# DIAGNijmegen/bodyct-dram-emph-subtype

Measured on NVIDIA B200. Metric: CT volumes/sec med3ddram inference, higher is better.
Workload: dtype f16 operands / f32 accumulate

## Files before the change

### bodyct-dram-emph-subtype_b200/csrc/common.h

```cpp
#pragma once
#include <cuda_bf16.h>
#include <cuda_fp16.h>
#include <cuda_runtime.h>
#include <stdarg.h>
#include <stdint.h>
#include <stdio.h>

#include "dram_b200.h"

namespace dram {

void set_error(const char *fmt, ...);

inline int check_cuda(cudaError_t e, const char *what) {
  if (e == cudaSuccess) return DRAM_OK;
  set_error("%s: %s", what, cudaGetErrorString(e));
  return DRAM_E_LAUNCH;
}

#define DRAM_REQUIRE(cond, ...)       \
  do {                                \
    if (!(cond)) {                    \
      ::dram::set_error(__VA_ARGS__); \
      return DRAM_E_ARG;              \
    }                                 \
  } while (0)

#define DRAM_CHECK_LAUNCH(what)                                       \
  do {                                                                \
    int _rc = ::dram::check_cuda(cudaGetLastError(), what);           \
    if (_rc != DRAM_OK) return _rc;                                   \
  } while (0)

inline int ceil_div(int a, int b) { return (a + b - 1) / b; }
inline int64_t ceil_div64(int64_t a, int64_t b) { return (a + b - 1) / b; }

int worklist_build(const uint32_t *bits, int n, int d, int h, int w, int tw, int th, int td, int d_fastest, int radius,
                   uint8_t *flags, int *list, int *count, int total, cudaStream_t st);

int sm_count();
inline int stream_grid(int64_t work_items, int threads, int ctas_per_sm = 8) {
  int64_t want = ceil_div64(work_items, threads);
  int64_t cap = (int64_t)sm_count() * ctas_per_sm;
  if (want < 1) want = 1;
  return (int)(want < cap ? want : cap);
}


#ifdef __CUDACC__
struct LinIdx {
  int i0, i1;
  float w0, w1;
};
__device__ __forceinline__ LinIdx lin_index_ac(int dst, float scale, int in_size) {
  LinIdx r;
  const float real = scale * (float)dst;
  int i0 = (int)real;
  if (i0 > in_size - 1) i0 = in_size - 1;
  r.i0 = i0;
  r.i1 = i0 + ((i0 < in_size - 1) ? 1 : 0);
  float l1 = real - (float)i0;
  l1 = fminf(fmaxf(l1, 0.0f), 1.0f);
  r.w1 = l1;
  r.w0 = 1.0f - l1;
  return r;
}
__device__ __forceinline__ float bilerp_hw(float a, float b, float c, float d, float w0, float w1, float h0, float h1) {
  return __fmaf_rn(h1, __fmaf_rn(w1, d, __fmul_rn(w0, c)), __fmul_rn(h0, __fmaf_rn(w1, b, __fmul_rn(w0, a))));
}
__device__ __forceinline__ float lerp_d(float p0, float p1, float d0, float d1) {
  return __fmaf_rn(d1, p1, __fmul_rn(d0, p0));
}
__host__ __device__ __forceinline__ float ac_scale(int in_size, int out_size) {
  return out_size > 1 ? (float)(in_size - 1) / (float)(out_size - 1) : 0.0f;
}
#endif

}
```

### bodyct-dram-emph-subtype_b200/csrc/conv3d_slab.cu

```cuda
#include <string.h>

#include "conv_plan.h"

namespace dram {

static constexpr int SL_W = 8, SL_H = 16;
__host__ __device__ constexpr int slab_group(int block_n) { return block_n == 128 ? 2 : 4; }
static constexpr int PL_W = SL_W + 2, PL_H = SL_H + 2;
static constexpr int PLANE_BYTES = PL_W * PL_H * 128;
static constexpr int PLANE_PITCH = 23 * 1024;
#ifndef DRAM_SLAB_RING
#define DRAM_SLAB_RING 7
#endif
static constexpr int RING = DRAM_SLAB_RING;
static constexpr int RING_UP = 6;
static constexpr int LP_W = 7, LP_H = 11;
static constexpr int LP_BYTES = LP_W * LP_H * 128;
static constexpr int LP_PITCH = 10 * 1024;
static constexpr int LP_RING = 3;
static constexpr int UP_WARP0 = 7, UP_THREADS = 128;
static constexpr int SL_THREADS = 224;
static constexpr int SL_A_WARP = 4, SL_MMA_WARP = 5, SL_B_WARP = 6;
static constexpr int SL_BLOCK_K = 64;

// ... 84 lines not shown
      mbar_init(plane_empty(s), 1);
    }
    for (int s = 0; s < B_STAGES; ++s) {
      mbar_init(b_full(s), 1);
      mbar_init(b_empty(s), 1);
    }
    for (int a = 0; a < 2; ++a) {
      mbar_init(tmem_full(a), 1);
      mbar_init(tmem_empty(a), 128);
    }
    if (UP)
      for (int s = 0; s < LP_RING; ++s) {
        mbar_init(lp_full(s), 1);
        mbar_init(lp_empty(s), UP_THREADS);
      }
    asm volatile("fence.mbarrier_init.release.cluster;" ::: "memory");
  }
  if (warp == SL_MMA_WARP) tmem_alloc(tmem_slot, Cfg::TMEM_COLS);
  if (warp == SL_A_WARP && lane == 0) {
    prefetch_tensormap(&map_a1);
    prefetch_tensormap(&map_a2);
  }
  if (warp == SL_B_WARP && lane == 0) prefetch_tensormap(&map_w);
  tcgen05_fence_before();
  __syncthreads();
  tcgen05_fence_after();
  uint32_t tmem_base;
  asm volatile("ld.shared.b32 %0, [%1];" : "=r"(tmem_base) : "r"(tmem_slot));
  tmem_base = __shfl_sync(0xffffffffu, tmem_base, 0);

  const int items_total = p.items ? *p.count : p.items_total;
  const int item_begin = (int)(((long long)blockIdx.x * items_total) / gridDim.x);
  const int item_end = (int)(((long long)(blockIdx.x + 1) * items_total) / gridDim.x);
  auto item_at = [&](int i) { return p.items ? __ldg(p.items + i) : i; };
  const bool single_chunk = !UP && p.chunks_total == 1;

  if (warp == SL_A_WARP) {
    if (lane == 0) {
      unsigned seq_end = 0;
      unsigned lseq = 0;
      int prev = -1;
      for (int i = item_begin; i < item_end; ++i) {
        const int item = item_at(i);
        const SlabItem it = decode_item(p, item, Cfg::GROUP);
        const bool reuse = single_chunk && prev == item - 1 && it.g > 0;
        prev = item;
        for (int c = 0; c < p.chunks_total; ++c) {
          const unsigned seq_base = seq_end - (reuse ? 2u : 0u);
          seq_end = seq_base + ITEM_PLANES;
          if (UP && c < p.chunks1) {
            const int zl0 = up_src_lo(it.q0 - 1, p.up_sd, p.Dl);
            const int zl1 = up_src_hi(it.q0 + SL_GROUP, p.D, p.up_sd, p.Dl);
            const int hl0 = up_src_lo(it.h0 - 1, p.up_sh, p.Hl), wl0 = up_src_lo(it.w0 - 1, p.up_sw, p.Wl);
            for (int zl = zl0; zl <= zl1; ++zl, ++lseq) {
              const int ls = lseq % LP_RING;
              mbar_wait(lp_empty(ls), ((lseq / LP_RING) & 1u) ^ 1u);
              mbar_expect_tx(lp_full(ls), LP_BYTES);
              tma_load_5d(lp_addr(ls), &map_a1, lp_full(ls), c * SL_BLOCK_K, wl0, hl0, zl, it.sample);
            }
            for (int j = 0; j < ITEM_PLANES; ++j) {
              const unsigned seq = seq_base + j;
              mbar_wait(plane_empty(seq % RING), ((seq / RING) & 1u) ^ 1u);
            }
            continue;
          }
          for (int j = reuse ? 2 : 0; j < ITEM_PLANES; ++j) {
            const unsigned seq = seq_base + j;
            const int slot = seq % RING;
            mbar_wait(plane_empty(slot), ((seq / RING) & 1u) ^ 1u);
            mbar_expect_tx(plane_full(slot), PLANE_BYTES);
            if (c < p.chunks1)
              tma_load_5d(plane_addr(slot), &map_a1, plane_full(slot), c * SL_BLOCK_K, it.w0 - 1, it.h0 - 1,
                          it.q0 - 1 + j, it.sample);
            else
              tma_load_5d(plane_addr(slot), &map_a2, plane_full(slot), (c - p.chunks1) * SL_BLOCK_K, it.w0 - 1,
                          it.h0 - 1, it.q0 - 1 + j, it.sample);
// ... 9 lines not shown
      for (int i = item_begin; i < item_end; ++i) {
        for (int c = 0; c < p.chunks_total; ++c) {
          for (int hw = 0; hw < 9; ++hw) {
            mbar_wait(b_empty(stage), phase ^ 1u);
            mbar_expect_tx(b_full(stage), Cfg::B_STAGE_BYTES);
#pragma unroll
            for (int blk = 0; blk < 3; ++blk) {
              const int tap = (2 - blk) * 9 + hw;
              tma_load_2d(b_addr(stage) + (uint32_t)(blk * Cfg::B_BLOCK_BYTES), &map_w, b_full(stage),
                          (tap * p.chunks_total + c) * SL_BLOCK_K, 0);
            }
            if (++stage == B_STAGES) {
              stage = 0;
              phase ^= 1u;
            }
          }
        }
      }
    }
    __syncwarp();
  } else if (warp == SL_MMA_WARP) {
    {
      uint32_t idesc[Cfg::MAX_BLK];
#pragma unroll
      for (int nb = 0; nb < Cfg::MAX_BLK; ++nb) idesc[nb] = make_idesc_16bit(128, (nb + 1) * BLOCK_N, p.epi.is_f16);
      const uint64_t desc_a_const = make_sw128_desc_sbo(0u, PL_W * 128, 0);
      const uint64_t desc_b_const = make_sw128_desc(0u);
      int stage = 0;
      uint32_t phase = 0;
      unsigned seq_end = 0;
      int buf = 0;
      uint32_t buf_phase = 0;
      int prev = -1;
      for (int i = item_begin; i < item_end; ++i) {
        const int item = item_at(i);
        const SlabItem it = decode_item(p, item, Cfg::GROUP);
        mbar_wait(tmem_empty(buf), buf_phase ^ 1u);
        tcgen05_fence_after();
        const uint32_t tmem_d0 = tmem_base + (uint32_t)(buf * SL_GROUP * BLOCK_N);
        const bool reuse = single_chunk && prev == item - 1 && it.g > 0;
        const bool next_reuse = single_chunk && i + 1 < item_end && it.g + 1 < p.groups_d && item_at(i + 1) == item + 1;
        prev = item;
        for (int c = 0; c < p.chunks_total; ++c) {
          const unsigned seq_base = seq_end - (reuse ? 2u : 0u);
          seq_end = seq_base + ITEM_PLANES;
          uint64_t da_plane[ITEM_PLANES];
          uint32_t full_bar[ITEM_PLANES], full_par[ITEM_PLANES], empty_bar[ITEM_PLANES];
#pragma unroll
          for (int j = 0; j < ITEM_PLANES; ++j) {
            const unsigned seq = seq_base + j;
            const int slot = seq % RING;
            uint32_t pa = plane_addr(slot);
            if (p.desc_base_offset_mode) pa |= 0u;
            pa = __shfl_sync(0xffffffffu, pa, 0);
            da_plane[j] = desc_a_const | (uint64_t)((pa & 0x3FFFFu) >> 4);
            full_bar[j] = plane_full(slot);
            full_par[j] = (seq / RING) & 1u;
            empty_bar[j] = plane_empty(slot);
          }
          const bool first_chunk = c == 0;
#pragma unroll
          for (int hw = 0; hw < 9; ++hw) {
            constexpr int kRowBytes = 128;
            const int kh = hw / 3, kw = hw - 3 * kh;
            const uint32_t row_off16 = (uint32_t)((kh * PL_W + kw) * kRowBytes) >> 4;
            mbar_wait(b_full(stage), phase);
            tcgen05_fence_after();
            uint32_t bb = b_addr(stage);
            bb = __shfl_sync(0xffffffffu, bb, 0);
            const uint64_t db_stage = desc_b_const | (uint64_t)((bb & 0x3FFFFu) >> 4);
            if (hw == 0) {
#pragma unroll
              for (int j = 0; j < ITEM_PLANES; ++j) {
                mbar_wait(full_bar[j], full_par[j]);
// ... 48 lines not shown
                    const uint64_t db = db_stage + (uint64_t)(((2 - kd_hi) * Cfg::B_BLOCK_BYTES) >> 4);
                    const uint32_t dcol = tmem_d0 + (uint32_t)(t_min * BLOCK_N);
                    umma_bf16(dcol, da + (uint64_t)(2 * k), db + (uint64_t)(2 * k), idesc[nblk - 1], 1u);
                  }
                }
                if (hw == 8) {
#pragma unroll
                  for (int j = 0; j < ITEM_PLANES; ++j)
                    if (j < SL_GROUP || !next_reuse) umma_commit(empty_bar[j]);
                }
                umma_commit(b_empty(stage));
              }
              __syncwarp();
            }
            if (++stage == B_STAGES) {
              stage = 0;
              phase ^= 1u;
            }
          }
        }
        if (elect_one_sync()) umma_commit(tmem_full(buf));
        __syncwarp();
        if (++buf == 2) {
          buf = 0;
          buf_phase ^= 1u;
        }
      }
    }
    __syncwarp();
  } else if (UP && warp >= UP_WARP0) {
    const int tid = threadIdx.x - UP_WARP0 * 32;
    const int is_f16 = p.epi.is_f16;
    unsigned seq_end = 0, lseq_base = 0;
    for (int i = item_begin; i < item_end; ++i) {
      const SlabItem it = decode_item(p, item_at(i), Cfg::GROUP);
      for (int c = 0; c < p.chunks_total; ++c) {
        const unsigned seq_base = seq_end;
        seq_end = seq_base + ITEM_PLANES;
        if (c >= p.chunks1) {
          for (int j = 0; j < ITEM_PLANES; ++j) {
            const unsigned seq = seq_base + j;
            mbar_wait(plane_empty(seq % RING), ((seq / RING) & 1u) ^ 1u);
          }
          continue;
        }
        const int zl0 = up_src_lo(it.q0 - 1, p.up_sd, p.Dl);
        const int zl1 = up_src_hi(it.q0 + SL_GROUP, p.D, p.up_sd, p.Dl);
        const int hl0 = up_src_lo(it.h0 - 1, p.up_sh, p.Hl), wl0 = up_src_lo(it.w0 - 1, p.up_sw, p.Wl);
        int released = zl0;
        for (int j = 0; j < ITEM_PLANES; ++j) {
          const unsigned seq = seq_base + j;
          const int slot = seq % RING;
          const int z = it.q0 - 1 + j;
          const bool zok = z >= 0 && z < p.D;
          mbar_wait(plane_empty(slot), ((seq / RING) & 1u) ^ 1u);
          LinIdx id = {0, 0, 0.0f, 0.0f};
          uint32_t lp0 = 0, lp1 = 0;
          if (zok) {
            id = lin_index_ac(z, p.up_sd, p.Dl);
            for (; released < id.i0; ++released) mbar_arrive(lp_empty((lseq_base + (unsigned)(released - zl0)) % LP_RING));
            const unsigned s0 = lseq_base + (unsigned)(id.i0 - zl0), s1 = lseq_base + (unsigned)(id.i1 - zl0);
            mbar_wait(lp_full(s0 % LP_RING), (s0 / LP_RING) & 1u);
            mbar_wait(lp_full(s1 % LP_RING), (s1 / LP_RING) & 1u);
            lp0 = lp_addr(s0 % LP_RING);
            lp1 = lp_addr(s1 % LP_RING);
          }
          const uint32_t dst0 = plane_addr(slot);
#pragma unroll 1
// ... 17 lines not shown
              lds(lp0 + o00, a0); lds(lp0 + o01, b0); lds(lp0 + o10, c0); lds(lp0 + o11, d0);
              lds(lp1 + o00, a1); lds(lp1 + o01, b1); lds(lp1 + o10, c1); lds(lp1 + o11, d1);
#pragma unroll
              for (int q = 0; q < 4; ++q) {
                const float2 fa0 = unpack2(a0[q], is_f16), fb0 = unpack2(b0[q], is_f16), fc0 = unpack2(c0[q], is_f16),
                             fd0 = unpack2(d0[q], is_f16);
                const float2 fa1 = unpack2(a1[q], is_f16), fb1 = unpack2(b1[q], is_f16), fc1 = unpack2(c1[q], is_f16),
                             fd1 = unpack2(d1[q], is_f16);
                const float x0 = bilerp_hw(fa0.x, fb0.x, fc0.x, fd0.x, iw.w0, iw.w1, ih.w0, ih.w1);
                const float x1 = bilerp_hw(fa1.x, fb1.x, fc1.x, fd1.x, iw.w0, iw.w1, ih.w0, ih.w1);
                const float y0 = bilerp_hw(fa0.y, fb0.y, fc0.y, fd0.y, iw.w0, iw.w1, ih.w0, ih.w1);
                const float y1 = bilerp_hw(fa1.y, fb1.y, fc1.y, fd1.y, iw.w0, iw.w1, ih.w0, ih.w1);
                o[q] = pack2(lerp_d(x0, x1, id.w0, id.w1), lerp_d(y0, y1, id.w0, id.w1), is_f16);
              }
            }
            const uint32_t dst = dst0 + (uint32_t)(r * 128) + (uint32_t)((c16 ^ (r & 7)) << 4);
            asm volatile("st.shared.v4.b32 [%0], {%1, %2, %3, %4};" ::"r"(dst), "r"(o[0]), "r"(o[1]), "r"(o[2]), "r"(o[3])
                         : "memory");
          }
          asm volatile("fence.proxy.async.shared::cta;" ::: "memory");
          asm volatile("bar.sync 1, %0;" ::"n"(UP_THREADS) : "memory");
          if (tid == 0) mbar_arrive(plane_full(slot));
        }
        for (; released <= zl1; ++released) mbar_arrive(lp_empty((lseq_base + (unsigned)(released - zl0)) % LP_RING));
        lseq_base += (unsigned)(zl1 - zl0 + 1);
      }
    }
  } else if (warp < 4) {
    const int row = warp * 32 + lane;
    const int lw = row & (SL_W - 1);
    const int lh = row >> 3;
    int buf = 0;
    uint32_t buf_phase = 0;
    for (int i = item_begin; i < item_end; ++i) {
      const SlabItem it = decode_item(p, item_at(i), Cfg::GROUP);
      const int oh = it.h0 + lh, ow = it.w0 + lw;
      auto res_ptr = [&](int t) {
        const int od = it.q0 + t;
        const bool valid = (od < p.D) && (oh < p.H) && (ow < p.W);
        return residual_row(p.epi, valid, it.sample, od, oh, ow);
      };
      constexpr int GROUPS_PER_PLANE = BLOCK_N / 32;
      ResGroup res = load_residual_group(p.epi, res_ptr(0), 0);
      mbar_wait(tmem_full(buf), buf_phase);
      tcgen05_fence_after();
#pragma unroll 1
      for (int t = 0; t < SL_GROUP; ++t) {
        const int od = it.q0 + t;
        const bool valid = (od < p.D) && (oh < p.H) && (ow < p.W);
        const uint16_t *res_row = res_ptr(t);
        const uint32_t taddr = tmem_base + (uint32_t)((buf * SL_GROUP + t) * BLOCK_N) + ((uint32_t)(warp * 32) << 16);
#pragma unroll 1
        for (int gq = 0; gq < GROUPS_PER_PLANE; ++gq) {
          const int c0 = gq * 32;
          uint32_t v[32];
          tmem_ld_32x32b_x32(taddr + (uint32_t)c0, v);
          ResGroup next;
          if (gq + 1 < GROUPS_PER_PLANE) next = load_residual_group(p.epi, res_row, c0 + 32);
          else next = load_residual_group(p.epi, t + 1 < SL_GROUP ? res_ptr(t + 1) : nullptr, 0);
          tmem_wait_ld();
#ifndef DRAM_SLAB_EXPERIMENT_NO_EPILOGUE
          if (valid) epilogue_group<BLOCK_N == 32>(p.epi, v, c0, it.sample, od, oh, ow, res);
#endif
          res = next;
        }
      }
      tcgen05_fence_before();
      mbar_arrive(tmem_empty(buf));
// ... 385 lines not shown
```

### bodyct-dram-emph-subtype_b200/csrc/decoder_mask.cu

```cuda
#include "common.h"

namespace dram {

__device__ __forceinline__ int first_source(int c, float scale, int out_size, int in_size) {
  if (c <= 0 || scale <= 0.0f) return 0;
  int x = (int)((float)c / scale);
  if (x > out_size - 1) x = out_size - 1;
  while (x > 0 && lin_index_ac(x - 1, scale, in_size).i0 >= c) --x;
  return x;
}

__global__ void __launch_bounds__(256)
support_rows_kernel(const uint8_t *__restrict__ ess, uint32_t *__restrict__ rows, int64_t total, int W, int w,
                    int words, float sw) {
  for (int64_t t = (int64_t)blockIdx.x * blockDim.x + threadIdx.x; t < total; t += (int64_t)gridDim.x * blockDim.x) {
    const int k = (int)(t % words);
    const uint8_t *e = ess + (t / words) * W;
    const int c0 = k * 32;
    uint32_t bits = 0;
    for (int x = first_source(c0 - 1, sw, W, w); x < W; ++x) {
      const LinIdx ix = lin_index_ac(x, sw, w);
      if (ix.i0 > c0 + 31) break;
      if (e[x]) {
        if (ix.i0 >= c0) bits |= 1u << (ix.i0 - c0);
        if (ix.i1 >= c0 && ix.i1 <= c0 + 31) bits |= 1u << (ix.i1 - c0);
      }
    }
    rows[t] = bits;
  }
}

__global__ void __launch_bounds__(256)
support_planes_kernel(const uint32_t *__restrict__ rows, uint32_t *__restrict__ bits, int n, int D, int H, int d,
                      int h, int words, float sd, float sh) {
  const int64_t total = (int64_t)n * d * h * words;
  for (int64_t t = (int64_t)blockIdx.x * blockDim.x + threadIdx.x; t < total; t += (int64_t)gridDim.x * blockDim.x) {
    const int k = (int)(t % words);
    int64_t r = t / words;
    const int y = (int)(r % h);
    r /= h;
    const int z = (int)(r % d);
    const int s = (int)(r / d);
    uint32_t acc = 0;
    for (int Z = first_source(z - 1, sd, D, d); Z < D; ++Z) {
      const LinIdx iz = lin_index_ac(Z, sd, d);
      if (iz.i0 > z) break;
      if (iz.i0 != z && iz.i1 != z) continue;
      for (int Y = first_source(y - 1, sh, H, h); Y < H; ++Y) {
        const LinIdx iy = lin_index_ac(Y, sh, h);
        if (iy.i0 > y) break;
        if (iy.i0 == y || iy.i1 == y) acc |= rows[(((int64_t)s * D + Z) * H + Y) * words + k];
      }
    }
    bits[t] = acc;
  }
}

__global__ void __launch_bounds__(256)
worklist_flags_kernel(const uint32_t *__restrict__ bits, uint8_t *__restrict__ flags, int total, int d, int h, int w,
                      int words, int tw, int th, int td, int d_fastest, int radius) {
  const int tiles_w = (w + tw - 1) / tw, tiles_h = (h + th - 1) / th, tiles_d = (d + td - 1) / td;
  for (int i = blockIdx.x * blockDim.x + threadIdx.x; i < total; i += gridDim.x * blockDim.x) {
    int r = i, iw, ih, id;
    if (d_fastest) {
      id = r % tiles_d; r /= tiles_d;
      iw = r % tiles_w; r /= tiles_w;
      ih = r % tiles_h; r /= tiles_h;
    } else {
      iw = r % tiles_w; r /= tiles_w;
      ih = r % tiles_h; r /= tiles_h;
      id = r % tiles_d; r /= tiles_d;
    }
    const int s = r;
    const int z0 = max(id * td - radius, 0), z1 = min(id * td + td - 1 + radius, d - 1);
    const int y0 = max(ih * th - radius, 0), y1 = min(ih * th + th - 1 + radius, h - 1);
    const int x0 = max(iw * tw - radius, 0), x1 = min(iw * tw + tw - 1 + radius, w - 1);
    const int k0 = x0 >> 5, k1 = x1 >> 5;
    bool on = false;
    for (int z = z0; z <= z1 && !on; ++z)
      for (int y = y0; y <= y1 && !on; ++y) {
        const uint32_t *row = bits + (((int64_t)s * d + z) * h + y) * words;
        for (int k = k0; k <= k1; ++k) {
          uint32_t m = 0xffffffffu;
          if (k == k0) m &= 0xffffffffu << (x0 & 31);
          if (k == k1) m &= 0xffffffffu >> (31 - (x1 & 31));
          if (row[k] & m) {
            on = true;
            break;
          }
        }
      }
    flags[i] = on ? 1 : 0;
  }
}

static constexpr int WL_THREADS = 1024, WL_PER_THREAD = 16;
__global__ void __launch_bounds__(WL_THREADS)
worklist_compact_kernel(const uint8_t *__restrict__ flags, int total, int *__restrict__ list, int *__restrict__ count) {
  __shared__ int warp_sum[WL_THREADS / 32];
  const int lane = threadIdx.x & 31, wid = threadIdx.x >> 5;
  int base = 0;
  for (int start = 0; start < total; start += WL_THREADS * WL_PER_THREAD) {
    const int i0 = start + threadIdx.x * WL_PER_THREAD;
    uint32_t m = 0;
#pragma unroll
    for (int j = 0; j < WL_PER_THREAD; ++j)
      if (i0 + j < total && flags[i0 + j]) m |= 1u << j;
    const int cnt = __popc(m);
    int incl = cnt;
#pragma unroll
    for (int o = 1; o < 32; o <<= 1) {
      const int v = __shfl_up_sync(0xffffffffu, incl, o);
      if (lane >= o) incl += v;
    }
    if (lane == 31) warp_sum[wid] = incl;
    __syncthreads();
    int before = 0, all = 0;
    for (int q = 0; q < WL_THREADS / 32; ++q) {
      const int v = warp_sum[q];
      if (q < wid) before += v;
      all += v;
    }
    int pos = base + before + incl - cnt;
    for (; m; m &= m - 1) list[pos++] = i0 + __ffs(m) - 1;
    base += all;
    __syncthreads();
  }
  if (threadIdx.x == 0) *count = base;
}

int worklist_build(const uint32_t *bits, int n, int d, int h, int w, int tw, int th, int td, int d_fastest, int radius,
                   uint8_t *flags, int *list, int *count, int total, cudaStream_t st) {
  if (!bits || !flags || !list || !count || n <= 0 || d <= 0 || h <= 0 || w <= 0 || total <= 0 || radius < 0) {
    set_error("worklist: null buffer, empty grid or negative radius");
    return DRAM_E_ARG;
  }
  const int words = ceil_div(w, 32);
  worklist_flags_kernel<<<ceil_div(total, 256) < 4096 ? ceil_div(total, 256) : 4096, 256, 0, st>>>(
      bits, flags, total, d, h, w, words, tw, th, td, d_fastest, radius);
  DRAM_CHECK_LAUNCH("worklist_flags_kernel launch");
  worklist_compact_kernel<<<1, WL_THREADS, 0, st>>>(flags, total, list, count);
  DRAM_CHECK_LAUNCH("worklist_compact_kernel launch");
  return DRAM_OK;
}

}

using namespace dram;

extern "C" int dram_decoder_support(const uint8_t *ess, int32_t n, int32_t D, int32_t H, int32_t W, int32_t d,
                                    int32_t h, int32_t w, uint32_t *rows, uint32_t *bits, void *stream) {
  DRAM_REQUIRE(ess && rows && bits, "dram_decoder_support: null pointer");
  DRAM_REQUIRE(n > 0 && D > 0 && H > 0 && W > 0 && d > 0 && h > 0 && w > 0 && d <= D && h <= H && w <= W,
               "dram_decoder_support: bad sizes (%d x %d x %d -> %d x %d x %d)", D, H, W, d, h, w);
  cudaStream_t st = reinterpret_cast<cudaStream_t>(stream);
  const int words = ceil_div(w, 32);
  const int64_t total_rows = (int64_t)n * D * H * words, total_bits = (int64_t)n * d * h * words;
  const int grid_rows = (int)(ceil_div64(total_rows, 256) < 8192 ? ceil_div64(total_rows, 256) : 8192);
  const int grid_bits = (int)(ceil_div64(total_bits, 256) < 8192 ? ceil_div64(total_bits, 256) : 8192);
  support_rows_kernel<<<grid_rows, 256, 0, st>>>(ess, rows, total_rows, W, w, words, ac_scale(w, W));
  DRAM_CHECK_LAUNCH("support_rows_kernel launch");
  support_planes_kernel<<<grid_bits, 256, 0, st>>>(rows, bits, n, D, H, d, h, words, ac_scale(d, D), ac_scale(h, H));
  DRAM_CHECK_LAUNCH("support_planes_kernel launch");
  return DRAM_OK;
}
```

### bodyct-dram-emph-subtype_b200/csrc/upsample_umma.cu

```cuda
#include "umma_common.cuh"

namespace dram {

static constexpr int U_TW = 8, U_TH = 4, U_TD = 4;
static constexpr int U_PW = 6, U_PH = 4, U_PD = 4;
static constexpr int U_K = U_PW * U_PH * U_PD;
static constexpr int U_B_BYTES = U_K * 128;
static constexpr int U_B_STAGES = 6;
static constexpr int U_W_BYTES = 2 * 128 * 128;
static constexpr int U_OUT_BYTES = 128 * 128;
static constexpr int U_ACC = 4;
static constexpr int U_THREADS = 320;
static constexpr int U_PRODUCER_WARP = 4, U_MMA_WARP = 5, U_GEN_WARP0 = 6;
static constexpr int U_SMEM_BYTES = 1024 + U_B_STAGES * U_B_BYTES + 2 * U_W_BYTES + 2 * U_OUT_BYTES + 256;

struct UpParams {
  int n, Dl, Hl, Wl, D, H, W, C;
  int chunks;
  int tiles_w, tiles_h, tiles_d, tiles_per_sample, total_tiles;
  float sd, sh, sw;
  int is_f16;
  const int *items, *count;
};

// ... 38 lines not shown
  auto w_empty = [&](int s) { return bar_base + 8u * (2 * U_B_STAGES + 2 + s); };
  auto t_full = [&](int a) { return bar_base + 8u * (2 * U_B_STAGES + 4 + a); };
  auto t_empty = [&](int a) { return bar_base + 8u * (2 * U_B_STAGES + 4 + U_ACC + a); };
  const uint32_t tmem_slot = bar_base + 8u * (2 * U_B_STAGES + 4 + 2 * U_ACC);

  const int warp = uniform_warp_idx();
  const int lane = threadIdx.x & 31;

  if (threadIdx.x == 0) {
    for (int s = 0; s < U_B_STAGES; ++s) {
      mbar_init(b_full(s), 1);
      mbar_init(b_empty(s), 1);
    }
    for (int s = 0; s < 2; ++s) {
      mbar_init(w_full(s), 128);
      mbar_init(w_empty(s), 1);
    }
    for (int a = 0; a < U_ACC; ++a) {
      mbar_init(t_full(a), 1);
      mbar_init(t_empty(a), 128);
    }
    asm volatile("fence.mbarrier_init.release.cluster;" ::: "memory");
  }
  if (warp == U_MMA_WARP) tmem_alloc(tmem_slot, U_ACC * 64);
  if (warp == U_PRODUCER_WARP && lane == 0) prefetch_tensormap(&map_in);
  if (threadIdx.x == 0) prefetch_tensormap(&map_out);
  tcgen05_fence_before();
  __syncthreads();
  tcgen05_fence_after();
  uint32_t tmem_base;
  asm volatile("ld.shared.b32 %0, [%1];" : "=r"(tmem_base) : "r"(tmem_slot));
  tmem_base = __shfl_sync(0xffffffffu, tmem_base, 0);
  const int total = p.items ? *p.count : p.total_tiles;
  auto tile_at = [&](int i) { return p.items ? __ldg(p.items + i) : i; };

  if (warp == U_PRODUCER_WARP) {
    if (lane == 0) {
      int stage = 0;
      uint32_t phase = 0;
      for (int i = blockIdx.x; i < total; i += gridDim.x) {
        const UpTile t = decode_up_tile(p, tile_at(i));
        for (int c = 0; c < p.chunks; ++c) {
          mbar_wait(b_empty(stage), phase ^ 1u);
          mbar_expect_tx(b_full(stage), U_B_BYTES);
          tma_load_5d(b_addr(stage), &map_in, b_full(stage), c * 64, t.wl0, t.hl0, t.dl0, t.sample);
          if (++stage == U_B_STAGES) {
            stage = 0;
            phase ^= 1u;
          }
        }
      }
    }
    __syncwarp();
  } else if (warp == U_MMA_WARP) {
    const uint32_t idesc = make_idesc_up(64, p.is_f16);
    int stage = 0, acc = 0, wi = 0;
    uint32_t phase = 0, acc_phase = 0, w_phase = 0;
    for (int i = blockIdx.x; i < total; i += gridDim.x) {
      mbar_wait(w_full(wi), w_phase);
      tcgen05_fence_after();
      for (int c = 0; c < p.chunks; ++c) {
        mbar_wait(t_empty(acc), acc_phase ^ 1u);
        mbar_wait(b_full(stage), phase);
        tcgen05_fence_after();
        if (elect_one_sync()) {
#pragma unroll
          for (int j = 0; j < U_K / 16; ++j) {
            const uint64_t da = make_sw128_desc(w_addr(wi) + (uint32_t)((j >> 2) * (128 * 128) + (j & 3) * 32));
            const uint64_t db = make_sw128_desc(b_addr(stage) + (uint32_t)(j * 16 * 128));
            umma_bf16(tmem_base + (uint32_t)(acc * 64), da, db, idesc, j > 0 ? 1u : 0u);
          }
          umma_commit(b_empty(stage));
          umma_commit(t_full(acc));
          if (c == p.chunks - 1) umma_commit(w_empty(wi));
// ... 36 lines not shown
        for (int a = 0; a < 3; ++a)
          if (ix[a].i1 == ix[a].i0) {
            ix[a].w0 += ix[a].w1;
            ix[a].w1 = 0.0f;
          }
#pragma unroll
        for (int cd = 0; cd < 2; ++cd)
#pragma unroll
          for (int chh = 0; chh < 2; ++chh)
#pragma unroll
            for (int cw = 0; cw < 2; ++cw) {
              const float wt = (cd ? ix[0].w1 : ix[0].w0) * ((chh ? ix[1].w1 : ix[1].w0) * (cw ? ix[2].w1 : ix[2].w0));
              if ((cd && ix[0].i1 == ix[0].i0) || (chh && ix[1].i1 == ix[1].i0) || (cw && ix[2].i1 == ix[2].i0)) continue;
              const int zd = (cd ? ix[0].i1 : ix[0].i0) - t.dl0, zh = (chh ? ix[1].i1 : ix[1].i0) - t.hl0;
              const int zw = (cw ? ix[2].i1 : ix[2].i0) - t.wl0;
              const int k = (zd * U_PH + zh) * U_PW + zw;
              const int kk = k & 63;
              const uint32_t addr = base + (uint32_t)((k >> 6) * 128 * 128) + (uint32_t)((((kk >> 3) ^ (r & 7)) << 4) + (kk & 7) * 2);
              unsigned short bits;
              if (p.is_f16) {
                const __half hv = __float2half_rn(wt);
                bits = *reinterpret_cast<const unsigned short *>(&hv);
              } else {
                const __nv_bfloat16 hv = __float2bfloat16_rn(wt);
                bits = *reinterpret_cast<const unsigned short *>(&hv);
              }
              asm volatile("st.shared.u16 [%0], %1;" ::"r"(addr), "h"(bits) : "memory");
              mine[cd * 4 + chh * 2 + cw] = addr;
            }
      }
    };
    int wi = 0;
    uint32_t w_phase = 0;
    for (int i = blockIdx.x; i < total; i += gridDim.x) {
      const UpTile t = decode_up_tile(p, tile_at(i));
      mbar_wait(w_empty(wi), w_phase ^ 1u);
      if (wi == 0) generate(t, w_addr(0), prev0);
      else generate(t, w_addr(1), prev1);
      asm volatile("fence.proxy.async.shared::cta;" ::: "memory");
      mbar_arrive(w_full(wi));
      if (++wi == 2) {
        wi = 0;
        w_phase ^= 1u;
      }
    }
  } else {
    const int row = warp * 32 + lane;
    int acc = 0, gi = 0;
    uint32_t acc_phase = 0;
    for (int i = blockIdx.x; i < total; i += gridDim.x) {
      const UpTile t = decode_up_tile(p, tile_at(i));
      for (int c = 0; c < p.chunks; ++c, ++gi) {
        const int b = gi & 1;
        mbar_wait(t_full(acc), acc_phase);
        tcgen05_fence_after();
        const uint32_t taddr = tmem_base + (uint32_t)(acc * 64) + ((uint32_t)(warp * 32) << 16);
        uint32_t v0[32], v1[32];
        tmem_ld_32x32b_x32(taddr, v0);
        tmem_ld_32x32b_x32(taddr + 32u, v1);
        if (threadIdx.x == 0) tma_store_wait_read<1>();
        asm volatile("bar.sync 1, 128;" ::: "memory");
        tmem_wait_ld();
        tcgen05_fence_before();
        mbar_arrive(t_empty(acc));
        const uint32_t orow = out_addr(b) + (uint32_t)row * 128u;
#pragma unroll
        for (int j = 0; j < 8; ++j) {
          const uint32_t *v = j < 4 ? v0 : v1;
          const int o = (j & 3) * 8;
          const uint32_t chunk = (uint32_t)((j ^ (row & 7)) << 4);
          asm volatile("st.shared.v4.b32 [%0], {%1, %2, %3, %4};" ::"r"(orow + chunk),
                       "r"(pack2(__uint_as_float(v[o + 0]), __uint_as_float(v[o + 1]), p.is_f16)),
                       "r"(pack2(__uint_as_float(v[o + 2]), __uint_as_float(v[o + 3]), p.is_f16)),
                       "r"(pack2(__uint_as_float(v[o + 4]), __uint_as_float(v[o + 5]), p.is_f16)),
                       "r"(pack2(__uint_as_float(v[o + 6]), __uint_as_float(v[o + 7]), p.is_f16))
                       : "memory");
        }
        asm volatile("fence.proxy.async.shared::cta;" ::: "memory");
        asm volatile("bar.sync 1, 128;" ::: "memory");
        if (threadIdx.x == 0) {
          tma_store_5d(&map_out, out_addr(b), c * 64, t.w0, t.h0, t.d0, t.sample);
          tma_store_commit();
        }
        if (++acc == U_ACC) {
// ... 125 lines not shown
```

### bodyct-dram-emph-subtype_b200/engine.py

```python
import os

import torch

from . import ops

LAYER_CFG = ((64, 1, 1), (128, 2, 1), (256, 1, 2), (512, 1, 4))


def _conv_out(n, k, s, d, p):
    return (n + 2 * p - d * (k - 1) - 1) // s + 1


class _Step:

    __slots__ = ("name", "fn", "flops", "executed_flops", "conv_part")

    def __init__(self, name, fn, flops=0, executed_flops=None, conv_part=False):
        self.name, self.fn, self.flops = name, fn, flops
        self.executed_flops = flops if executed_flops is None else executed_flops
        self.conv_part = conv_part or flops > 0


class Med3DEngine:
    def __init__(self, model, batch, dims, device, act_dtype=None):
        if device.type != "cuda":
            raise RuntimeError("Med3DEngine needs a CUDA device: this path has no CPU implementation")
        self.model = model
        self.act_dtype = ops.default_act_dtype() if act_dtype is None else act_dtype
        self.batch, self.dims, self.device = batch, tuple(dims), device
        self.head_kind = model.head_kind
        self._weights = {}
        self._packers = []
        self.steps = []
        self.conv_flops = 0
        self._graph = None
        self._graph_restricted = None
        self._restricted = None
        self._sat_counter = torch.zeros(1, dtype=torch.int32, device=device)
        self._sat_checked_epoch = None
        self.last_saturation_count = None
        self._build()
        self._weights_epoch = model.weights_epoch


    def _register_weight(self, name, pack_fn):
        bufs = tuple(t.to(self.device).contiguous() for t in pack_fn())
        self._weights[name] = bufs

        def refill(bufs=bufs, pack_fn=pack_fn):
            for dst, src in zip(bufs, pack_fn()):
                dst.copy_(src)

        self._packers.append(refill)
# ... 180 lines not shown
        self.us1_g = torch.empty((B, D2, H2, W2, 64), dtype=bf, device=dev)
        self.steps.append(_Step("us1.0.gather_w", lambda: ops.upconv_axis(z, 3, 9, out=self.us1_r), conv_part=True))
        self.steps.append(_Step("us1.0.gather_h", lambda: ops.upconv_axis(self.us1_r, 2, 3, out=self.us1_q), conv_part=True))
        self.steps.append(_Step("us1.0.gather_d", lambda: ops.upconv_axis(self.us1_q, 1, 1, out=self.us1_g), conv_part=True))
        wskip = self._register_weight("us1.0.skip", pack_skip)
        return self._add_conv("us1.0", x1, wskip, residual=self.us1_g).out

    def _launch_steps(self, first=None):
        (first or self.steps[0].fn)()
        self._launch_tail()

    def _launch_tail(self):
        for st in self.steps[1:]:
            st.fn()

    def hu_stem(self, hu, lut, lo=-1150):
        if not hasattr(self, "stem_weights"):
            raise RuntimeError("the int16-HU stem needs the fused stem kernel (DRAM_B200_STEM=unfold is set)")
        if tuple(hu.shape) != (self.batch,) + self.dims:
            raise ValueError(f"hu shape {tuple(hu.shape)} does not match the engine's {(self.batch,) + self.dims}")
        w, b, m = self.stem_weights
        return lambda: ops.stem_conv7_hu(hu, lut, w, b, m, out=self.stem_out, lo=lo)

    def image_stem(self, image):
        if not hasattr(self, "stem_weights"):
            raise RuntimeError("image_stem needs the fused stem kernel (DRAM_B200_STEM=unfold is set)")
        img = image.reshape(self.batch, *self.dims)
        if img.dtype != torch.float32 or not img.is_contiguous():
            raise ValueError("image_stem: expected a contiguous fp32 image")
        w, b, m = self.stem_weights
        return lambda: ops.stem_conv7(img, w, b, m, out=self.stem_out)

    def _restricted_tail(self):
        for fn in self._restricted[2]:
            fn()

    def _support(self, ess):
        if tuple(ess.shape) != (self.batch,) + self.dims or ess.dtype != torch.uint8 or not ess.is_contiguous():
            raise ValueError(f"active_ess: expected contiguous uint8 {(self.batch,) + self.dims}, got "
                             f"{ess.dtype} {tuple(ess.shape)}")
        if self._restricted is None:
            B, (D, H, W), (d, h, w) = self.batch, self.dims, self.half_dims
            words = (w + 31) // 32
            rows = torch.empty((B, D, H, words), dtype=torch.int32, device=self.device)
            support = torch.empty((B, d, h, words), dtype=torch.int32, device=self.device)
            lists, listed = [], {}
            for name, plan, radius, _ in self._decoder:
                size = plan.worklist_size() if plan is not None else 0
                if size == 0:
                    continue
                flags = torch.empty(size, dtype=torch.uint8, device=self.device)
                items = torch.empty(size, dtype=torch.int32, device=self.device)
                count = torch.empty(1, dtype=torch.int32, device=self.device)
                lists.append(lambda plan=plan, r=radius, f=flags, i=items, c=count: plan.build_worklist(support, r, f, i, c))
                listed[name] = lambda plan=plan, i=items, c=count: plan.run_listed(i, c)
            self._restricted = (rows, support, lists + [listed.get(st.name, st.fn) for st in self.steps[1:]])
        rows, support, _ = self._restricted
        ops.decoder_support(ess, self.half_dims, rows=rows, out=support)

    def run_network(self, first=None, active_ess=None):
        if self._weights_epoch != self.model.weights_epoch:
            self.refresh_weights()
        mode = ops.sat_check_mode()
        if self.act_dtype == torch.float16 and (
                mode == "always" or (mode == "first" and self._sat_checked_epoch != self._weights_epoch)):
            lib = ops._capi.load()
            self._sat_counter.zero_()
            ops.check(lib.dram_set_saturation_counter(ops._p(self._sat_counter)), "dram_set_saturation_counter")
            try:
                self._launch_steps(first)
            finally:
                lib.dram_set_saturation_counter(None)
            clamped = int(self._sat_counter.item())
            self.last_saturation_count = clamped
            if clamped:
                raise ops.ActivationOverflow(
                    f"{clamped} 32-channel output groups exceeded the fp16 range (+-65504) and were clamped: this "
                    "checkpoint/input needs bf16 storage (model.act_dtype = torch.bfloat16 or DRAM_B200_DTYPE=bf16)")
            self._sat_checked_epoch = self._weights_epoch
            return self.dense
        tail = self._launch_tail
        if active_ess is not None:
            self._support(active_ess)
            tail = self._restricted_tail
        if not ops.graphs_enabled() or torch.cuda.is_current_stream_capturing():
            (first or self.steps[0].fn)()
            tail()
            return self.dense
        (first or self.steps[0].fn)()
        attr = "_graph" if active_ess is None else "_graph_restricted"
        if getattr(self, attr) is None:
# ... 34 lines not shown
```

Before: 221.6.

## Overlap worklist builds on side stream and parallelise decoder support kernels

The restricted-decoder path now builds its worklists on a side CUDA stream, letting them overlap the encoder steps, and joins the main stream just before the first listed step. The worklist compaction moves from one CTA to a multi-CTA scan. The support-row bitmask kernel now reads the ess mask with vectorised 16-byte loads, skips zero vectors and accumulates bits in shared memory with atomics. Item-list prefetching via a cursor struct and hoisting one loop bound are smaller tweaks. These changes add stream-synchronisation complexity and a dependence on the side stream being captured correctly in graphs.

```diff
diff --git a/bodyct-dram-emph-subtype_b200/csrc/common.h b/bodyct-dram-emph-subtype_b200/csrc/common.h
--- a/bodyct-dram-emph-subtype_b200/csrc/common.h
+++ b/bodyct-dram-emph-subtype_b200/csrc/common.h
@@ -48,6 +48,23 @@
 
 
 #ifdef __CUDACC__
+struct ListCursor {
+  const int *items;
+  int pos, end, stride, cur, nxt;
+  __device__ __forceinline__ int at(int i) const { return i < end ? (items ? __ldg(items + i) : i) : -1; }
+  __device__ __forceinline__ ListCursor(const int *list, int begin, int end_, int stride_ = 1)
+      : items(list), pos(begin), end(end_), stride(stride_) {
+    cur = at(begin);
+    nxt = at(begin + stride_);
+  }
+  __device__ __forceinline__ bool more() const { return pos < end; }
+  __device__ __forceinline__ void next() {
+    pos += stride;
+    cur = nxt;
+    nxt = at(pos + stride);
+  }
+};
+
 struct LinIdx {
   int i0, i1;
   float w0, w1;
diff --git a/bodyct-dram-emph-subtype_b200/csrc/conv3d_slab.cu b/bodyct-dram-emph-subtype_b200/csrc/conv3d_slab.cu
--- a/bodyct-dram-emph-subtype_b200/csrc/conv3d_slab.cu
+++ b/bodyct-dram-emph-subtype_b200/csrc/conv3d_slab.cu
@@ -140,7 +140,6 @@
   const int items_total = p.items ? *p.count : p.items_total;
   const int item_begin = (int)(((long long)blockIdx.x * items_total) / gridDim.x);
   const int item_end = (int)(((long long)(blockIdx.x + 1) * items_total) / gridDim.x);
-  auto item_at = [&](int i) { return p.items ? __ldg(p.items + i) : i; };
   const bool single_chunk = !UP && p.chunks_total == 1;
 
   if (warp == SL_A_WARP) {
@@ -148,8 +147,8 @@
       unsigned seq_end = 0;
       unsigned lseq = 0;
       int prev = -1;
-      for (int i = item_begin; i < item_end; ++i) {
-        const int item = item_at(i);
+      for (ListCursor lc(p.items, item_begin, item_end); lc.more(); lc.next()) {
+        const int item = lc.cur;
         const SlabItem it = decode_item(p, item, Cfg::GROUP);
         const bool reuse = single_chunk && prev == item - 1 && it.g > 0;
         prev = item;
@@ -225,14 +224,14 @@
       int buf = 0;
       uint32_t buf_phase = 0;
       int prev = -1;
-      for (int i = item_begin; i < item_end; ++i) {
-        const int item = item_at(i);
+      for (ListCursor lc(p.items, item_begin, item_end); lc.more(); lc.next()) {
+        const int item = lc.cur;
         const SlabItem it = decode_item(p, item, Cfg::GROUP);
         mbar_wait(tmem_empty(buf), buf_phase ^ 1u);
         tcgen05_fence_after();
         const uint32_t tmem_d0 = tmem_base + (uint32_t)(buf * SL_GROUP * BLOCK_N);
         const bool reuse = single_chunk && prev == item - 1 && it.g > 0;
-        const bool next_reuse = single_chunk && i + 1 < item_end && it.g + 1 < p.groups_d && item_at(i + 1) == item + 1;
+        const bool next_reuse = single_chunk && it.g + 1 < p.groups_d && lc.nxt == item + 1;
         prev = item;
         for (int c = 0; c < p.chunks_total; ++c) {
           const unsigned seq_base = seq_end - (reuse ? 2u : 0u);
@@ -347,8 +346,8 @@
     const int tid = threadIdx.x - UP_WARP0 * 32;
     const int is_f16 = p.epi.is_f16;
     unsigned seq_end = 0, lseq_base = 0;
-    for (int i = item_begin; i < item_end; ++i) {
-      const SlabItem it = decode_item(p, item_at(i), Cfg::GROUP);
+    for (ListCursor lc(p.items, item_begin, item_end); lc.more(); lc.next()) {
+      const SlabItem it = decode_item(p, lc.cur, Cfg::GROUP);
       for (int c = 0; c < p.chunks_total; ++c) {
         const unsigned seq_base = seq_end;
         seq_end = seq_base + ITEM_PLANES;
@@ -432,8 +431,8 @@
     const int lh = row >> 3;
     int buf = 0;
     uint32_t buf_phase = 0;
-    for (int i = item_begin; i < item_end; ++i) {
-      const SlabItem it = decode_item(p, item_at(i), Cfg::GROUP);
+    for (ListCursor lc(p.items, item_begin, item_end); lc.more(); lc.next()) {
+      const SlabItem it = decode_item(p, lc.cur, Cfg::GROUP);
       const int oh = it.h0 + lh, ow = it.w0 + lw;
       auto res_ptr = [&](int t) {
         const int od = it.q0 + t;
diff --git a/bodyct-dram-emph-subtype_b200/csrc/decoder_mask.cu b/bodyct-dram-emph-subtype_b200/csrc/decoder_mask.cu
--- a/bodyct-dram-emph-subtype_b200/csrc/decoder_mask.cu
+++ b/bodyct-dram-emph-subtype_b200/csrc/decoder_mask.cu
@@ -10,24 +10,82 @@
   return x;
 }
 
-__global__ void __launch_bounds__(256)
-support_rows_kernel(const uint8_t *__restrict__ ess, uint32_t *__restrict__ rows, int64_t total, int W, int w,
-                    int words, float sw) {
-  for (int64_t t = (int64_t)blockIdx.x * blockDim.x + threadIdx.x; t < total; t += (int64_t)gridDim.x * blockDim.x) {
-    const int k = (int)(t % words);
-    const uint8_t *e = ess + (t / words) * W;
-    const int c0 = k * 32;
-    uint32_t bits = 0;
-    for (int x = first_source(c0 - 1, sw, W, w); x < W; ++x) {
-      const LinIdx ix = lin_index_ac(x, sw, w);
-      if (ix.i0 > c0 + 31) break;
-      if (e[x]) {
-        if (ix.i0 >= c0) bits |= 1u << (ix.i0 - c0);
-        if (ix.i1 >= c0 && ix.i1 <= c0 + 31) bits |= 1u << (ix.i1 - c0);
+static constexpr int SUP_THREADS = 256, SUP_VECS = 4;
+static constexpr int SUP_SPAN = SUP_THREADS * SUP_VECS * 16;
+
+struct SupportWindow {
+  int r = -1, base = 0;
+  uint64_t m = 0;
+
+  __device__ __forceinline__ void flush(uint32_t *acc, int words) {
+    if (!m) return;
+    uint32_t *row = acc + r * words + (base >> 5);
+    atomicOr(row, (uint32_t)m);
+    if (m >> 32) atomicOr(row + 1, (uint32_t)(m >> 32));
+    m = 0;
+  }
+  __device__ __forceinline__ void mark(uint32_t *acc, int words, int row, int x, float sw, int w) {
+    const LinIdx ix = lin_index_ac(x, sw, w);
+    if (row != r) {
+      flush(acc, words);
+      r = row;
+      base = ix.i0 & ~31;
+    }
+    m |= (1ull << (ix.i0 - base)) | (1ull << (ix.i1 - base));
+  }
+};
+
+__global__ void __launch_bounds__(SUP_THREADS)
+support_rows_kernel(const uint8_t *__restrict__ ess, uint32_t *__restrict__ rows, int64_t total_rows,
+                    int rows_per_cta, int W, int w, int words, float sw) {
+  extern __shared__ uint32_t acc[];
+  const int64_t r0 = (int64_t)blockIdx.x * rows_per_cta;
+  const int nr = (int)(total_rows - r0 < rows_per_cta ? total_rows - r0 : rows_per_cta);
+  for (int i = threadIdx.x; i < nr * words; i += SUP_THREADS) acc[i] = 0;
+  __syncthreads();
+  const uint8_t *span = ess + r0 * W;
+  const int len = nr * W;
+  const int head = min((int)((16 - (reinterpret_cast<uintptr_t>(span) & 15)) & 15), len);
+  const int nvec = (len - head) >> 4, tail = head + nvec * 16;
+  {
+    SupportWindow win;
+    const int p = threadIdx.x;
+    if (p < head && span[p]) win.mark(acc, words, p / W, p % W, sw, w);
+    win.flush(acc, words);
+    const int q = tail + threadIdx.x;
+    if (q < len && span[q]) win.mark(acc, words, q / W, q % W, sw, w);
+    win.flush(acc, words);
+  }
+  const uint4 *vec = reinterpret_cast<const uint4 *>(span + head);
+  for (int i0 = 0; i0 < nvec; i0 += SUP_THREADS * SUP_VECS) {
+    uint4 v[SUP_VECS];
+#pragma unroll
+    for (int k = 0; k < SUP_VECS; ++k) {
+      const int i = i0 + k * SUP_THREADS + threadIdx.x;
+      v[k] = i < nvec ? __ldg(vec + i) : make_uint4(0, 0, 0, 0);
+    }
+#pragma unroll
+    for (int k = 0; k < SUP_VECS; ++k) {
+      if (!(v[k].x | v[k].y | v[k].z | v[k].w)) continue;
+      const uint32_t q[4] = {v[k].x, v[k].y, v[k].z, v[k].w};
+      const int p = head + (i0 + k * SUP_THREADS + threadIdx.x) * 16;
+      const int r = p / W, x = p - r * W;
+      const bool one_row = x + 16 <= W;
+      SupportWindow win;
+#pragma unroll
+      for (int c = 0; c < 4; ++c) {
+        for (uint32_t nz = (((q[c] & 0x7f7f7f7fu) + 0x7f7f7f7fu) | q[c]) & 0x80808080u; nz; nz &= nz - 1) {
+          const int xj = x + 4 * c + ((__ffs(nz) - 1) >> 3);
+          if (one_row) win.mark(acc, words, r, xj, sw, w);
+          else win.mark(acc, words, r + xj / W, xj % W, sw, w);
+        }
       }
-    }
-    rows[t] = bits;
-  }
+      win.flush(acc, words);
+    }
+  }
+  __syncthreads();
+  uint32_t *out = rows + r0 * words;
+  for (int i = threadIdx.x; i < nr * words; i += SUP_THREADS) out[i] = acc[i];
 }
 
 __global__ void __launch_bounds__(256)
@@ -42,11 +100,12 @@
     const int z = (int)(r % d);
     const int s = (int)(r / d);
     uint32_t acc = 0;
+    const int y_first = first_source(y - 1, sh, H, h);
     for (int Z = first_source(z - 1, sd, D, d); Z < D; ++Z) {
       const LinIdx iz = lin_index_ac(Z, sd, d);
       if (iz.i0 > z) break;
       if (iz.i0 != z && iz.i1 != z) continue;
-      for (int Y = first_source(y - 1, sh, H, h); Y < H; ++Y) {
+      for (int Y = y_first; Y < H; ++Y) {
         const LinIdx iy = lin_index_ac(Y, sh, h);
         if (iy.i0 > y) break;
         if (iy.i0 == y || iy.i1 == y) acc |= rows[(((int64_t)s * D + Z) * H + Y) * words + k];
@@ -94,39 +153,55 @@
   }
 }
 
-static constexpr int WL_THREADS = 1024, WL_PER_THREAD = 16;
+static constexpr int WL_THREADS = 256, WL_PER_THREAD = 16, WL_CHUNK = WL_THREADS * WL_PER_THREAD;
+
+__device__ __forceinline__ int block_exclusive_sum(int v, int *all) {
+  __shared__ int warp_sum[WL_THREADS / 32];
+  const int lane = threadIdx.x & 31, wid = threadIdx.x >> 5;
+  int incl = v;
+#pragma unroll
+  for (int o = 1; o < 32; o <<= 1) {
+    const int u = __shfl_up_sync(0xffffffffu, incl, o);
+    if (lane >= o) incl += u;
+  }
+  if (lane == 31) warp_sum[wid] = incl;
+  __syncthreads();
+  int before = 0, sum = 0;
+#pragma unroll
+  for (int q = 0; q < WL_THREADS / 32; ++q) {
+    const int u = warp_sum[q];
+    if (q < wid) before += u;
+    sum += u;
+  }
+  *all = sum;
+  return before + incl - v;
+}
+
 __global__ void __launch_bounds__(WL_THREADS)
 worklist_compact_kernel(const uint8_t *__restrict__ flags, int total, int *__restrict__ list, int *__restrict__ count) {
-  __shared__ int warp_sum[WL_THREADS / 32];
-  const int lane = threadIdx.x & 31, wid = threadIdx.x >> 5;
-  int base = 0;
-  for (int start = 0; start < total; start += WL_THREADS * WL_PER_THREAD) {
-    const int i0 = start + threadIdx.x * WL_PER_THREAD;
-    uint32_t m = 0;
-#pragma unroll
-    for (int j = 0; j < WL_PER_THREAD; ++j)
-      if (i0 + j < total && flags[i0 + j]) m |= 1u << j;
-    const int cnt = __popc(m);
-    int incl = cnt;
-#pragma unroll
-    for (int o = 1; o < 32; o <<= 1) {
-      const int v = __shfl_up_sync(0xffffffffu, incl, o);
-      if (lane >= o) incl += v;
-    }
-    if (lane == 31) warp_sum[wid] = incl;
-    __syncthreads();
-    int before = 0, all = 0;
-    for (int q = 0; q < WL_THREADS / 32; ++q) {
-      const int v = warp_sum[q];
-      if (q < wid) before += v;
-      all += v;
-    }
-    int pos = base + before + incl - cnt;
-    for (; m; m &= m - 1) list[pos++] = i0 + __ffs(m) - 1;
-    base += all;
-    __syncthreads();
-  }
-  if (threadIdx.x == 0) *count = base;
+  const int start = blockIdx.x * WL_CHUNK;
+  int ahead = 0;
+  const int head = min((int)((16 - (reinterpret_cast<uintptr_t>(flags) & 15)) & 15), start);
+  const int nvec = (start - head) >> 4;
+  if ((int)threadIdx.x < head) ahead += flags[threadIdx.x];
+  if (head + nvec * 16 + (int)threadIdx.x < start) ahead += flags[head + nvec * 16 + threadIdx.x];
+  const uint4 *vec = reinterpret_cast<const uint4 *>(flags + head);
+  for (int i = threadIdx.x; i < nvec; i += WL_THREADS) {
+    const uint4 v = __ldg(vec + i);
+    ahead += __popc(v.x) + __popc(v.y) + __popc(v.z) + __popc(v.w);
+  }
+  int all_ahead;
+  block_exclusive_sum(ahead, &all_ahead);
+  __syncthreads();
+  const int i0 = start + threadIdx.x * WL_PER_THREAD;
+  uint32_t m = 0;
+#pragma unroll
+  for (int j = 0; j < WL_PER_THREAD; ++j)
+    if (i0 + j < total && flags[i0 + j]) m |= 1u << j;
+  int in_chunk;
+  int pos = all_ahead + block_exclusive_sum(__popc(m), &in_chunk);
+  for (; m; m &= m - 1) list[pos++] = i0 + __ffs(m) - 1;
+  if (blockIdx.x == gridDim.x - 1 && threadIdx.x == 0) *count = all_ahead + in_chunk;
 }
 
 int worklist_build(const uint32_t *bits, int n, int d, int h, int w, int tw, int th, int td, int d_fastest, int radius,
@@ -139,7 +214,7 @@
   worklist_flags_kernel<<<ceil_div(total, 256) < 4096 ? ceil_div(total, 256) : 4096, 256, 0, st>>>(
       bits, flags, total, d, h, w, words, tw, th, td, d_fastest, radius);
   DRAM_CHECK_LAUNCH("worklist_flags_kernel launch");
-  worklist_compact_kernel<<<1, WL_THREADS, 0, st>>>(flags, total, list, count);
+  worklist_compact_kernel<<<ceil_div(total, WL_CHUNK), WL_THREADS, 0, st>>>(flags, total, list, count);
   DRAM_CHECK_LAUNCH("worklist_compact_kernel launch");
   return DRAM_OK;
 }
@@ -155,10 +230,15 @@
                "dram_decoder_support: bad sizes (%d x %d x %d -> %d x %d x %d)", D, H, W, d, h, w);
   cudaStream_t st = reinterpret_cast<cudaStream_t>(stream);
   const int words = ceil_div(w, 32);
-  const int64_t total_rows = (int64_t)n * D * H * words, total_bits = (int64_t)n * d * h * words;
-  const int grid_rows = (int)(ceil_div64(total_rows, 256) < 8192 ? ceil_div64(total_rows, 256) : 8192);
+  DRAM_REQUIRE((int64_t)words * 4 <= 48 * 1024, "dram_decoder_support: w = %d is too wide", w);
+  const int64_t ess_rows = (int64_t)n * D * H, total_bits = (int64_t)n * d * h * words;
+  int rows_per_cta = W < SUP_SPAN ? SUP_SPAN / W : 1;
+  if (rows_per_cta * words * 4 > 48 * 1024) rows_per_cta = 48 * 1024 / (words * 4);
+  const int64_t grid_rows = ceil_div64(ess_rows, rows_per_cta);
+  DRAM_REQUIRE(grid_rows < (1ll << 31), "dram_decoder_support: ess too large");
   const int grid_bits = (int)(ceil_div64(total_bits, 256) < 8192 ? ceil_div64(total_bits, 256) : 8192);
-  support_rows_kernel<<<grid_rows, 256, 0, st>>>(ess, rows, total_rows, W, w, words, ac_scale(w, W));
+  support_rows_kernel<<<(unsigned)grid_rows, SUP_THREADS, (size_t)rows_per_cta * words * 4, st>>>(
+      ess, rows, ess_rows, rows_per_cta, W, w, words, ac_scale(w, W));
   DRAM_CHECK_LAUNCH("support_rows_kernel launch");
   support_planes_kernel<<<grid_bits, 256, 0, st>>>(rows, bits, n, D, H, d, h, words, ac_scale(d, D), ac_scale(h, H));
   DRAM_CHECK_LAUNCH("support_planes_kernel launch");
diff --git a/bodyct-dram-emph-subtype_b200/csrc/upsample_umma.cu b/bodyct-dram-emph-subtype_b200/csrc/upsample_umma.cu
--- a/bodyct-dram-emph-subtype_b200/csrc/upsample_umma.cu
+++ b/bodyct-dram-emph-subtype_b200/csrc/upsample_umma.cu
@@ -94,14 +94,13 @@
   asm volatile("ld.shared.b32 %0, [%1];" : "=r"(tmem_base) : "r"(tmem_slot));
   tmem_base = __shfl_sync(0xffffffffu, tmem_base, 0);
   const int total = p.items ? *p.count : p.total_tiles;
-  auto tile_at = [&](int i) { return p.items ? __ldg(p.items + i) : i; };
 
   if (warp == U_PRODUCER_WARP) {
     if (lane == 0) {
       int stage = 0;
       uint32_t phase = 0;
-      for (int i = blockIdx.x; i < total; i += gridDim.x) {
-        const UpTile t = decode_up_tile(p, tile_at(i));
+      for (ListCursor lc(p.items, blockIdx.x, total, gridDim.x); lc.more(); lc.next()) {
+        const UpTile t = decode_up_tile(p, lc.cur);
         for (int c = 0; c < p.chunks; ++c) {
           mbar_wait(b_empty(stage), phase ^ 1u);
           mbar_expect_tx(b_full(stage), U_B_BYTES);
@@ -204,8 +203,8 @@
     };
     int wi = 0;
     uint32_t w_phase = 0;
-    for (int i = blockIdx.x; i < total; i += gridDim.x) {
-      const UpTile t = decode_up_tile(p, tile_at(i));
+    for (ListCursor lc(p.items, blockIdx.x, total, gridDim.x); lc.more(); lc.next()) {
+      const UpTile t = decode_up_tile(p, lc.cur);
       mbar_wait(w_empty(wi), w_phase ^ 1u);
       if (wi == 0) generate(t, w_addr(0), prev0);
       else generate(t, w_addr(1), prev1);
@@ -220,8 +219,8 @@
     const int row = warp * 32 + lane;
     int acc = 0, gi = 0;
     uint32_t acc_phase = 0;
-    for (int i = blockIdx.x; i < total; i += gridDim.x) {
-      const UpTile t = decode_up_tile(p, tile_at(i));
+    for (ListCursor lc(p.items, blockIdx.x, total, gridDim.x); lc.more(); lc.next()) {
+      const UpTile t = decode_up_tile(p, lc.cur);
       for (int c = 0; c < p.chunks; ++c, ++gi) {
         const int b = gi & 1;
         mbar_wait(t_full(acc), acc_phase);
diff --git a/bodyct-dram-emph-subtype_b200/engine.py b/bodyct-dram-emph-subtype_b200/engine.py
--- a/bodyct-dram-emph-subtype_b200/engine.py
+++ b/bodyct-dram-emph-subtype_b200/engine.py
@@ -19,6 +19,14 @@
         self.name, self.fn, self.flops = name, fn, flops
         self.executed_flops = flops if executed_flops is None else executed_flops
         self.conv_part = conv_part or flops > 0
+
+
+class _Restricted:
+
+    def __init__(self):
+        self.rows = self.support = self.side = None
+        self.builds, self.lists, self.steps = [], [], []
+        self.join_at = None
 
 
 class Med3DEngine:
@@ -265,7 +273,16 @@
         return lambda: ops.stem_conv7(img, w, b, m, out=self.stem_out)
 
     def _restricted_tail(self):
-        for fn in self._restricted[2]:
+        r = self._restricted
+        main = torch.cuda.current_stream(self.device)
+        if r.builds:
+            r.side.wait_stream(main)
+            with torch.cuda.stream(r.side):
+                for build in r.builds:
+                    build()
+        for i, fn in enumerate(r.steps):
+            if i == r.join_at:
+                main.wait_stream(r.side)
             fn()
 
     def _support(self, ess):
@@ -275,9 +292,11 @@
         if self._restricted is None:
             B, (D, H, W), (d, h, w) = self.batch, self.dims, self.half_dims
             words = (w + 31) // 32
-            rows = torch.empty((B, D, H, words), dtype=torch.int32, device=self.device)
-            support = torch.empty((B, d, h, words), dtype=torch.int32, device=self.device)
-            lists, listed = [], {}
+            r = _Restricted()
+            r.rows = torch.empty((B, D, H, words), dtype=torch.int32, device=self.device)
+            r.support = torch.empty((B, d, h, words), dtype=torch.int32, device=self.device)
+            r.side = torch.cuda.Stream(self.device)
+            listed = {}
             for name, plan, radius, _ in self._decoder:
                 size = plan.worklist_size() if plan is not None else 0
                 if size == 0:
@@ -285,11 +304,15 @@
                 flags = torch.empty(size, dtype=torch.uint8, device=self.device)
                 items = torch.empty(size, dtype=torch.int32, device=self.device)
                 count = torch.empty(1, dtype=torch.int32, device=self.device)
-                lists.append(lambda plan=plan, r=radius, f=flags, i=items, c=count: plan.build_worklist(support, r, f, i, c))
+                r.builds.append(lambda plan=plan, s=r.support, rad=radius, f=flags, i=items, c=count:
+                                plan.build_worklist(s, rad, f, i, c))
+                r.lists.append((name, items, count))
                 listed[name] = lambda plan=plan, i=items, c=count: plan.run_listed(i, c)
-            self._restricted = (rows, support, lists + [listed.get(st.name, st.fn) for st in self.steps[1:]])
-        rows, support, _ = self._restricted
-        ops.decoder_support(ess, self.half_dims, rows=rows, out=support)
+            r.steps = [listed.get(st.name, st.fn) for st in self.steps[1:]]
+            names = [st.name for st in self.steps[1:]]
+            r.join_at = min((names.index(n) for n in listed), default=None)
+            self._restricted = r
+        ops.decoder_support(ess, self.half_dims, rows=self._restricted.rows, out=self._restricted.support)
 
     def run_network(self, first=None, active_ess=None):
         if self._weights_epoch != self.model.weights_epoch:
```

Measured after the change: 224.3 (median of 6 runs). 1.01x the previous value.
